# abiswas-odu/Disco

Hardware: AMD Instinct MI355X
Metric: overlaps/sec (BuildGraph stage), 150 bp reads (higher is better)
Workload: dtype u64; 1 GPU; 50000000 x 150 bp synthetic reads, 30x of 50 x 5000000 bp uniform-random contigs, both strands, error-free, min-overlap 40 (k=39), transitive reduction on, seed 42; reads=50000000, read_len=150, min_overlap=40, parallelism=1 GPU, e_pre=903537181, e_out=45314794, n_contained=4685156, cap_bind_sites=0, asymmetric_pairs=0, probes=5550000000, kmer_hits=2220071992

## Files before the change

disco_amd/csrc/disco_hip.hip:

```cpp
#include <hip/hip_runtime.h>
#include <rocprofiler-sdk-roctx/roctx.h>

#include <algorithm>
#include <atomic>
#include <chrono>
#include <cstdarg>
#include <cstdio>
#include <cstdlib>
#include <cstring>
#include <fcntl.h>
#include <sys/mman.h>
#include <sys/stat.h>
#include <unistd.h>
#include <string>
#include <memory>
#include <thread>
#include <map>
#include <mutex>
#include <vector>

#include "../../include/disco_hip.h"
#include "../../include/disco_hip_test.h"
#include "../../include/disco_hip_inspect.h"
#include "disco_kernels.h"
// ... 844 lines not shown
    c->runs_by_pos = false;
    const int nf = v.k - v.m + 1;
    const int lpr = c->S == VERIFY_SW ? runs_lpr_for(c, nf, c->max_len, nloc) : 0;
    if (lpr && nloc) {
        CHK(ensure(c, c->d_runs, nloc * (u64)lpr));
        c->runs_lpr = lpr;
        c->runs_lo = lo;
        c->runs_n = nloc;
        c->runs_by_pos = list != nullptr;
        pl->lpr = lpr;
        pl->nf = nf;
    }
    return DISCO_OK;
}

typedef void (*IndexRunsFn)(DiscoView, u32 *, ulonglong2 *, u32 *, u64, u64, u32 *, u32 *, u32 *, u64 *, u32, u32, const u64 *);
typedef void (*IndexCountFn)(DiscoView, u32 *, ulonglong2 *, u32 *, u64, u64, u32 *, u32 *, u64 *, u32, u32, const u64 *);
struct IndexCountKernel {
    IndexRunsFn runs = nullptr;
    IndexCountFn plain = nullptr;
};
template <bool COUNT, int NF, int NFMAX, bool LONGK>
static IndexCountKernel index_runs_pick(int lpr)
{
    IndexCountKernel k;
    k.runs = lpr == 16 ? index_runs_kernel<COUNT, NF, 1, NFMAX, LONGK> : index_runs_kernel<COUNT, NF, 2, NFMAX, LONGK>;
    return k;
}
template <bool COUNT>
static IndexCountKernel index_count_pick(int nf, int m, int lpr, bool longk, bool long_class)
{
    if (long_class || !lpr) {
        IndexCountKernel k;
        if (long_class) k.plain = longk ? index_count_kernel<COUNT, true, true> : index_count_kernel<COUNT, false, true>;
        else k.plain = longk ? index_count_kernel<COUNT, true> : index_count_kernel<COUNT>;
        return k;
    }
    if (runs_nf_built(nf, m)) switch (nf) {
        case 7: return index_runs_pick<COUNT, 7, 7, false>(lpr);
        case 12: return index_runs_pick<COUNT, 12, 12, false>(lpr);
        case 17: return index_runs_pick<COUNT, 17, 17, false>(lpr);
        case 22: return index_runs_pick<COUNT, 22, 22, false>(lpr);
        default: return index_runs_pick<COUNT, 27, 27, false>(lpr);
        }
    if (longk) return nf <= 48 ? index_runs_pick<COUNT, 0, 48, true>(lpr) : index_runs_pick<COUNT, 0, 64, true>(lpr);
    if (nf <= 8) return index_runs_pick<COUNT, 0, 8, false>(lpr);
    if (nf <= 12) return index_runs_pick<COUNT, 0, 12, false>(lpr);
    if (nf <= 16) return index_runs_pick<COUNT, 0, 16, false>(lpr);
    if (nf <= 24) return index_runs_pick<COUNT, 0, 24, false>(lpr);
    if (nf <= 32) return index_runs_pick<COUNT, 0, 32, false>(lpr);
    if (nf <= 48) return index_runs_pick<COUNT, 0, 48, false>(lpr);
    return index_runs_pick<COUNT, 0, 64, false>(lpr);
}
static IndexCountKernel index_count_pick(bool count, int nf, int m, int lpr, bool longk, bool long_class)
{
    return count ? index_count_pick<true>(nf, m, lpr, longk, long_class) : index_count_pick<false>(nf, m, lpr, longk, long_class);
}

static int index_count_chunk(disco_ctx *c, const DiscoView &v, const IndexCountPlan &pl, bool count, ulonglong2 *rec_base, u64 a, u64 b)
{
    if (b <= a) return DISCO_OK;
    const dim3 grid((unsigned)((b - a + 255) / 256));
    ulonglong2 *rec = rec_base + 2 * (a - pl.lo);
    u32 *oslot = pl.oslot ? pl.oslot + (a - pl.lo) : nullptr;
    u64 *oitem = pl.oitem ? pl.oitem + (a - pl.lo) : nullptr;
    u32 *okey = pl.list ? nullptr : c->d_okey.p;
    const IndexCountKernel k = index_count_pick(count, pl.nf, v.m, pl.lpr, c->k > 64, false);
    if (k.runs) hipLaunchKernelGGL(k.runs, grid, dim3(256), 0, c->stream, v, c->d_bkt, rec, okey, a, b, c->d_runs + (a - pl.lo) * (u64)pl.lpr, pl.ocnt, oslot, oitem, pl.oidbits, pl.oshift, pl.list);
    else hipLaunchKernelGGL(k.plain, grid, dim3(256), 0, c->stream, v, c->d_bkt, rec, okey, a, b, pl.ocnt, oslot, oitem, pl.oidbits, pl.oshift, pl.list);
    HIPCHK(c, hipGetLastError());
    return DISCO_OK;
}

static int index_count_long(disco_ctx *c, const DiscoView &v, const IndexCountPlan &pl, bool count, ulonglong2 *rec, u32 *oslot, u64 x_lo, u64 x_hi)
{
    const dim3 g((unsigned)((x_hi - x_lo + 255) / 256));
    hipLaunchKernelGGL(index_count_pick(count, 0, v.m, 0, c->k > 64, true).plain, g, dim3(256), 0, c->stream, v, c->d_bkt, rec, c->d_okey, x_lo, x_hi, pl.ocnt, oslot, (u64 *)nullptr, 0u, pl.oshift,
                       (const u64 *)nullptr);
    HIPCHK(c, hipGetLastError());
    return DISCO_OK;
}

static bool binned_index_wanted(disco_ctx *c, int logT)
{
    if (getenv("DISCO_NO_BINNED_INDEX") || 2 * c->n >= 0xFFFF0000ull) return false;
    if (logT > BINX_SPAN_BITS && ensure(c, c->d_rec2, 2 * c->n) != DISCO_OK) {
        (void)hipGetLastError();
        c->err.clear();
        return false;
    }
    return true;
}

static int size_bucket_table(disco_ctx *c)
{
    u64 T = 1024;
    int logT = 10;
    double tscale = 2.0;
    if (const char *e = getenv("DISCO_BUCKET_SCALE")) tscale = atof(e);
    while ((double)T < tscale * (double)c->n && logT < 32) {
        T <<= 1;
        logT++;
    }
    c->T = T;
    c->bshift = 64 - logT;
    return logT;
}

static int index_begin(disco_ctx *c)
{
    const int logT = size_bucket_table(c);
    const u64 T = c->T;
    CHK(ensure(c, c->d_bkt, T + 1));
    CHK(ensure(c, c->d_ent, 2 * c->n));
    CHK(ensure(c, c->d_rec, 2 * c->n));
    CHK(ensure(c, c->d_okey, c->n));
    c->adj_imported = false;
    c->binned_index = binned_index_wanted(c, logT);
    if (!c->binned_index) HIPCHK(c, hipMemsetAsync(c->d_bkt, 0, (T + 1) * sizeof(u32), c->stream));
    return DISCO_OK;
}

struct BinxPlan {
    int span = 0, levels = 0, bits[3] = {0, 0, 0};
};
static BinxPlan binx_plan(int logT)
{
    BinxPlan b;
    b.span = std::min(logT, BINX_SPAN_BITS);
    const int prefix = logT - b.span;
    b.levels = (prefix + BINX_MAX_BITS - 1) / BINX_MAX_BITS;
    for (int l = 0; l < b.levels; l++) b.bits[l] = prefix / b.levels + (l < prefix % b.levels ? 1 : 0);
    return b;
}

template <typename R>
static int binx_partition(disco_ctx *c, const char *what, int bits, u32 kshift, u32 total, R *src, R *dst, const R **out, const u32 **part)
{
    const BinxPlan bp = binx_plan(bits);
    const u32 n_part = 1u << (bits - bp.span);
    const u32 tiles = (total + BINX_TILE - 1u) / BINX_TILE;
    u64 hist_len = 1;
    for (int l = 0, done = 0; l < bp.levels; done += bp.bits[l], l++) hist_len = std::max<u64>(hist_len, ((u64)tiles + (1ull << done)) * (1ull << bp.bits[l]) + 1);
    const u64 tab = ((u64)n_part + 1 + 63) & ~63ull;
    CHK(ensure(c, c->d_binx, 4 * tab + hist_len));
    u32 *seg[2] = {c->d_binx.p, c->d_binx.p + tab}, *tb[2] = {c->d_binx.p + 2 * tab, c->d_binx.p + 3 * tab}, *hist = c->d_binx.p + 4 * tab;
    if (getenv("DISCO_VERBOSE"))
        fprintf(stderr, "[disco] binned %s: 2^%d buckets, %u partitions of 2^%d, %d level(s) of %d / %d / %d bits\n", what, bits, n_part, bp.span, bp.levels, bp.bits[0], bp.bits[1], bp.bits[2]);
    u32 pseg = 1, pnb = 1;
    int cur = 0, done = 0;
    for (int l = 0; l < bp.levels; l++) {
        const u32 nseg = 1u << done, nb = 1u << bp.bits[l], shift = kshift + (u32)(bits - done - bp.bits[l]);
        const u32 grid = tiles + nseg;
        const u64 hlen = (u64)grid * nb + 1;
        hipLaunchKernelGGL(binx_segs_kernel, dim3(1), dim3(1024), 0, c->stream, l ? (const u32 *)hist : (const u32 *)nullptr, (const u32 *)tb[cur ^ 1], pseg, pnb, total, seg[cur], tb[cur]);
        HIPCHK(c, hipMemsetAsync(hist, 0, hlen * sizeof(u32), c->stream));
        hipLaunchKernelGGL(binx_hist_kernel<R>, dim3(grid), dim3(BINX_BLOCK), 0, c->stream, (const R *)src, (const u32 *)seg[cur], (const u32 *)tb[cur], nseg, shift, nb, hist);
        CHK((scan_exclusive<u32, u32>(c, hist, hlen, hist, false, nullptr)));
        hipLaunchKernelGGL(binx_scatter_kernel<R>, dim3(grid), dim3(BINX_BLOCK), 0, c->stream, (const R *)src, dst, (const u32 *)seg[cur], (const u32 *)tb[cur], nseg, shift, nb, (const u32 *)hist);
        HIPCHK(c, hipGetLastError());
        std::swap(src, dst);
        pseg = nseg;
        pnb = nb;
        done += bp.bits[l];
        cur ^= 1;
    }
    hipLaunchKernelGGL(binx_segs_kernel, dim3(1), dim3(1024), 0, c->stream, bp.levels ? (const u32 *)hist : (const u32 *)nullptr, (const u32 *)tb[cur ^ 1], pseg, pnb, total, seg[cur],
                       (u32 *)nullptr);
    HIPCHK(c, hipGetLastError());
    *out = src;
    *part = seg[cur];
    return DISCO_OK;
}

static int binned_build_index(disco_ctx *c)
{
    const int logT = 64 - c->bshift;
    const u32 total = (u32)(2 * c->n);
    const ulonglong2 *rec;
    const u32 *part;
    CHK(binx_partition(c, "index build", logT, 32u, total, c->d_rec.p, c->d_rec2.p, &rec, &part));
    const int span = std::min(logT, BINX_SPAN_BITS);
    hipLaunchKernelGGL(binx_build_kernel<ulonglong2>, dim3(1u << (logT - span)), dim3(BINX_BUILD_BLOCK), 0, c->stream, rec, part, (u32)span, 32u, 0u, total, c->T, c->d_bkt.p, c->d_ent.p);
    HIPCHK(c, hipGetLastError());
    return DISCO_OK;
}

static int binned_build_order(disco_ctx *c)
{
    const int bits = c->order_counted_bits;
    const u32 total = (u32)c->n, kshift = 64u - (u32)bits;
    u64 *items = (u64 *)c->d_rec2.p;
    const u64 *rec;
    const u32 *part;
    CHK(binx_partition(c, "grouping", bits, kshift, total, items, items + c->n, &rec, &part));
    const int span = std::min(bits, BINX_SPAN_BITS);
    hipLaunchKernelGGL(binx_build_kernel<u64>, dim3(1u << (bits - span)), dim3(BINX_BUILD_BLOCK), 0, c->stream, rec, part, (u32)span, kshift, (u32)c->order_id_bits, total, (u64)0,
                       (u32 *)nullptr, c->d_order_own.p);
    HIPCHK(c, hipGetLastError());
    return DISCO_OK;
}

static int start_contained_rows(disco_ctx *c, bool grouped)
{
    const u64 nc = c->n_contained;
    if (c->crows_pending && c->crows_n == nc && (!grouped || c->cgrp_pending)) return DISCO_OK;
    const bool have_rows = c->crows_pending && c->crows_n == nc;
    if (!have_rows) c->crows_pending = c->cgrp_pending = false;
    const u64 max_rows = getenv("DISCO_EAGER_ROWS_MAX") ? (u64)atoll(getenv("DISCO_EAGER_ROWS_MAX")) : (16ull << 20);
    if (c->comm || nc == 0 || nc > max_rows || c->n >= (1ull << 31)) return DISCO_OK;
    if (!c->aux_stream) {
        HIPCHK(c, hipStreamCreateWithFlags(&c->aux_stream, hipStreamNonBlocking));
// ... 614 lines not shown
                if (k >= 3) HIPCHK(c, hipStreamWaitEvent(c->copy_stream, c->ev_unpacked[b], 0));
                HIPCHK(c, hipMemcpyAsync(ring, packed + w0, (w1 - w0) * 8, hipMemcpyHostToDevice, c->copy_stream));
                HIPCHK(c, hipEventRecord(c->ev_copied[b], c->copy_stream));
                HIPCHK(c, hipStreamWaitEvent(c->stream, c->ev_copied[b], 0));
                hipLaunchKernelGGL(unpack_reads_kernel, dim3(flat_grid(c, (hi - lo) * (u64)c->S)), dim3(256), 0, c->stream, (const u64 *)ring, ragged ? 0 : (int)stride_words, (const u64 *)woff, w0,
                                   (const u16 *)c->d_len, lo, hi, c->S, classes ? (u32)DISCO_SHORT_MAX : 0xFFFFu, c->d_reads);
                if (classes)
                    hipLaunchKernelGGL(unpack_long_reads_kernel, dim3(flat_grid(c, shape.n_long * ((u64)dstride + 8))), dim3(256), 0, c->stream, (const u64 *)ring, ragged ? 0 : (int)stride_words,
                                       (const u64 *)woff, w0, (const u16 *)c->d_len, lo, hi, (const u32 *)c->d_long_ids, shape.n_long, n, (int)dstride, c->tailb, c->d_full, c->d_reads);
                HIPCHK(c, hipEventRecord(c->ev_unpacked[b], c->stream));
            } else {
                HIPCHK(c, hipMemcpyAsync(c->d_reads + lo * dstride, packed + lo * dstride, (hi - lo) * (u64)dstride * 8, hipMemcpyHostToDevice, c->copy_stream));
                HIPCHK(c, hipEventRecord(c->ev_copied[b], c->copy_stream));
                HIPCHK(c, hipStreamWaitEvent(c->stream, c->ev_copied[b], 0));
            }
            if (eager) CHK(index_count_chunk(c, v, pl, !c->binned_index, c->d_rec, lo, hi));
        }
        HIPCHK(c, hipGetLastError());
        t_issued = lapms();
        if (c->h_len.size() != n) c->h_len.resize(n);
        uint16_t *hl = c->h_len.data();
        parallel_for(n, [&, hl](u64 b0, u64 e0) { memcpy(hl + b0, len + b0, (e0 - b0) * 2); });
        c->h_len_ok = true;
        t_mirror = lapms();
        HIPCHK(c, hipStreamSynchronize(c->copy_stream));
        if (getenv("DISCO_VERBOSE"))
            fprintf(stderr, "[disco] %s: lengths checked %.1f ms, buffers %.1f, chunks issued %.1f, lengths mirrored %.1f, copies done %.1f (%s%s)\n", who, t_scan, t_alloc, t_issued,
                    t_mirror, lapms(), classes ? "two classes of rows" : "one stride", eager ? ", index counted behind the copies" : "");
        if (woff) {
            HIPCHK(c, hipStreamSynchronize(c->stream));
            release(c, woff);
// ... 909 lines not shown
int disco_build_index(disco_ctx *c)
{
    DISCO_TRACE("disco_build_index");
    if (!c) return DISCO_E_ARG;
    if (c->phase < 1) return fail(c, DISCO_E_STATE, "disco_build_index: no reads");
    HIPCHK(c, hipSetDevice(c->device));
    ph_begin(c, DISCO_PH_INDEX);
    if (c->index_counted) {
        c->index_counted = false;
    } else {
        CHK(two_class_convert(c));
        CHK(index_begin(c));
        const DiscoView v = view(c);
        IndexCountPlan pl;
        CHK(index_count_plan(c, v, 0, c->n, &pl));
        CHK(index_count_chunk(c, v, pl, !c->binned_index, c->d_rec, 0, c->n));
        if (c->two_class) CHK(index_count_long(c, v, pl, !c->binned_index, c->d_rec, pl.oslot, 0, c->n_long));
    }
    const bool binned = c->binned_index;
    if (!binned) CHK((scan_exclusive<u32, u32>(c, c->d_bkt, c->T + 1, c->d_bkt, false, nullptr)));
    c->order_ready = false;
    if (c->order_counted && c->order_counted_lo == 0 && c->order_counted_hi == c->n && !c->two_class && !getenv("DISCO_NO_ORDERED_FILL")) {
        const u64 order_buckets = 1ull << c->order_counted_bits;
        CHK(ensure(c, c->d_order_own, c->n));
        ph_end(c, DISCO_PH_INDEX);
        ph_begin(c, DISCO_PH_ORDER);
        if (c->order_items) CHK(binned_build_order(c));
        else {
            CHK((scan_exclusive<u32, u32>(c, c->d_ocnt, order_buckets + 1, c->d_ocnt, false, nullptr)));
            hipLaunchKernelGGL(order_scatter_kernel, dim3(flat_grid(c, c->n)), dim3(256), 0, c->stream, c->d_okey, c->d_oslot, c->d_ocnt, 32u - (u32)c->order_counted_bits, (u64)0, c->n, c->d_len, c->d_order_own);
        }
        ph_end(c, DISCO_PH_ORDER);
// ... 1904 lines not shown
    auto blo_of = [&](u64 g) { return (g * T + G - 1) / G; };
    const u64 blo = blo_of(r), bhi = blo_of(r + 1);
    const bool part = c->part_index;
    if (!part) {
        CHK(ensure(c, c->d_bkt, T + 1));
        CHK(ensure(c, c->d_ent, 2 * c->n));
    }
    CHK(ensure(c, c->d_okey, c->loci ? c->n_alloc : c->n));
    CHK(ensure(c, c->d_rec, std::max<u64>(2 * nloc, 1)));
    c->adj_imported = false;
    ph_begin(c, DISCO_PH_INDEX);
    DiscoView v = view(c);
    IndexCountPlan pl;
    if (c->loci) {
        CHK(index_count_plan(c, v, 0, c->n_own, &pl, c->d_order_own));
        CHK(index_count_chunk(c, v, pl, false, c->d_rec, 0, c->n_own));
    } else {
        CHK(index_count_plan(c, v, c->q_lo, c->q_hi, &pl));
        CHK(index_count_chunk(c, v, pl, false, c->d_rec, c->q_lo, c->q_hi));
        if (c->two_class && nloc) {
            u32 xb[2] = {0, (u32)c->n_long};
            HIPCHK(c, hipMemcpyAsync(&xb[0], c->d_ovf + c->q_lo, sizeof(u32), hipMemcpyDeviceToHost, c->stream));
            if (c->q_hi < c->n) HIPCHK(c, hipMemcpyAsync(&xb[1], c->d_ovf + c->q_hi, sizeof(u32), hipMemcpyDeviceToHost, c->stream));
            HIPCHK(c, hipStreamSynchronize(c->stream));
            if (xb[1] > xb[0]) {
                ulonglong2 *rec_by_id = c->d_rec - 2 * (ptrdiff_t)c->q_lo;
                u32 *oslot_by_id = pl.oslot ? pl.oslot - (ptrdiff_t)c->q_lo : nullptr;
                CHK(index_count_long(c, v, pl, false, rec_by_id, oslot_by_id, xb[0], xb[1]));
            }
        }
    }
    CHK(ensure(c, c->d_x16a, std::max<u64>(2 * nloc, 1)));
    std::vector<u64> scnt, rcnt, matrix;
    RouteByBucket f{logT, G};
    CHK(route_items(c, c->d_rec.p, 2 * nloc, f, c->d_x16a.p, scnt));
    CHK(exchange_counts(c, scnt, rcnt, &matrix));
    const u64 nrec = vsum(rcnt);
    CHK(ensure(c, c->d_x16b, std::max<u64>(nrec, 1)));
    CHK(a2a_items(c, DISCO_X_INDEX_RECORDS, c->d_x16a, scnt, c->d_x16b, rcnt, sizeof(ulonglong2)));
    std::vector<u64> shard((size_t)G, 0);
    for (u32 p = 0; p < G; p++)
        for (u32 q = 0; q < G; q++) shard[q] += matrix[(size_t)p * G + q];
    u64 base = 0;
// ... 1353 lines not shown
```

disco_amd/csrc/disco_kernels.h:

```cpp
#ifndef DISCO_KERNELS_H_
#define DISCO_KERNELS_H_

#include "disco_device.h"
#include "readgen.h"

#define PROBE_ROWCAP 512
#define PROBE_SEGW 128
#define PROBE_SEGP (PROBE_SEGW + 64)
#define PROBE_ACAP 32
#define PROBE_CHUNK 4096
#define ES_MID 1024
#define ES_DUPBITS 11
#define ES_DUPTAB (1 << ES_DUPBITS)
#ifndef ES_CAP
#define ES_CAP 256
#endif
#ifndef TR_CAP
#define TR_CAP 256
#endif
#define TR_CAP_SMALL 128
#define VERIFY_SW 8
#define ORDER_BUCKET(key, shift) (((key) * 0x9E3779B1u) >> (shift))
#define SCAN_ITEMS 16
#define SCAN_BLOCK 256
// ... 187 lines not shown
        if (L <= (u32)min_overlap || L > 32767u || L > (u32)S * 32u) bad++;
        mx = L > mx ? L : mx;
        mn = L < mn ? L : mn;
    }
    if (bad) atomicAdd(&ctr[CTR_BAD_LEN], (u64)bad);
    for (int o = 32; o > 0; o >>= 1) {
        mx = max(mx, (u32)__shfl_down(mx, o));
        mn = min(mn, (u32)__shfl_down(mn, o));
    }
    if ((threadIdx.x & 63) == 0) {
        atomicMax(&ctr[CTR_MAX_LEN], (u64)mx);
        atomicMax(&ctr[CTR_MIN_LEN], (u64)(0xFFFFu - mn));
    }
}

template <bool COUNT, bool LONGK = false, bool LONGCLASS = false>
__global__ void __launch_bounds__(256) index_count_kernel(DiscoView v, u32 *__restrict__ bkt, ulonglong2 *__restrict__ rec, u32 *__restrict__ okey, u64 lo, u64 hi,
                                                          u32 *__restrict__ ocnt, u32 *__restrict__ oslot, u64 *__restrict__ oitem, u32 oidbits, u32 oshift,
                                                          const u64 *__restrict__ list = nullptr)
{
    const u64 x = lo + (u64)blockIdx.x * 256u + threadIdx.x;
    if (x >= hi) return;
    const u64 i = LONGCLASS ? (u64)v.long_ids[x] : x;
    const u64 lw = (!LONGCLASS && list) ? list[x] : 0ull;
    const u64 rid = (!LONGCLASS && list) ? ORDER_ID(lw) : i;
    if (LONGCLASS) lo = 0;
    const int S = LONGCLASS ? v.SL : v.S;
    const u64 *__restrict__ p = LONGCLASS ? v.full + x * (u64)S : v.reads + rid * (u64)S;
    if (!LONGCLASS && v.full && v.len[rid] > DISCO_SHORT_MAX) return;
    const int L = (!LONGCLASS && list) ? ORDER_LEN(lw) : (int)v.len[rid], k = v.k, m = v.m, nf = k - m + 1;
    const int nmm = L - m + 1;
    const int sfx0 = nmm - nf;
    const u64 mask = (1ull << (2 * m)) - 1ull;
// ... 41 lines not shown
        const int ffirst = (int)((k1 >> 1) & 63u), flast = 63 - (int)((k2 >> 1) & 63u);
        int fsel = ffirst;
        if (ffirst == flast)
            rev = k1 & 1u;
        else {
            rev = kmer_is_rev<false, LONGK>(p, S, j0, k);
            fsel = rev ? flast : ffirst;
        }
        t = rev ? (u32)(nf - 1 - fsel) : (u32)fsel;
        return mmer_key(p, S, j0 + fsel, m);
    };
    u32 tp, rp, ts, rs;
    const u64 kp = resolve(k1p, k2p, 0, tp, rp);
    const u64 ks = resolve(k1s, k2s, sfx0, ts, rs);
    const u64 bp = kp >> v.bshift, bs = ks >> v.bshift;
    const u32 sp = COUNT ? atomicAdd(&bkt[bp], 1u) : 0u;
    const u32 ss = COUNT ? atomicAdd(&bkt[bs], 1u) : 0u;
    rec[2 * (i - lo)] = make_ulonglong2((bp << 32) | sp, PAY_MAKE(kp, rid, tp, rp, 0, L));
    rec[2 * (i - lo) + 1] = make_ulonglong2((bs << 32) | ss, PAY_MAKE(ks, LONGCLASS ? v.n + x : rid, ts, rs, 1, L));
}

#define RUNS_M 23
template <bool B>
struct FlagConst {
    static constexpr bool value = B;
};
template <int M>
struct MmerRoll {
    static_assert(M == 0 || (M > 16 && M <= 24 && (M & 1)), "two dwords, the high one partly used; a 24-bit fold in order_hash32<false>");
    const u64 *__restrict__ p;
    int last_word;
    u32 himask, rsh;
    int pos = 0;
    u64 word = 0;
// ... 19 lines not shown
        chi = st ? rhi : fhi;
    }
    __device__ __forceinline__ u32 hash() const { return order_hash32<M == 0>(((u64)chi << 32) | clo); }
    __device__ __forceinline__ u32 strand() const { return st ? 1u : 0u; }
};
#define RUN_W(e) ((u32)(e) >> 7)
#define RUN_DELTA(e) (((u32)(e) >> 1) & 63u)
#define RUN_STRAND(e) ((u32)(e)&1u)
#define OCC_MAKE(slot, e, wend) (((u32)(slot) << 29) | (RUN_STRAND(e) << 23) | (RUN_DELTA(e) << 17) | ((u32)(wend) << 8) | RUN_W(e))
#define OCC_SLOT(d) ((u32)(d) >> 29)
#define OCC_STRAND(d) (((u32)(d) >> 23) & 1u)
#define OCC_DELTA(d) (((u32)(d) >> 17) & 63u)
#define OCC_END(d) (((u32)(d) >> 8) & 0x1FFu)
#define OCC_FIRST(d) ((u32)(d)&0xFFu)

template <bool COUNT, int NF, int NL, int NFMAX = NF, bool LONGK = false>
__global__ void __launch_bounds__(256) index_runs_kernel(DiscoView v, u32 *__restrict__ bkt, ulonglong2 *__restrict__ rec, u32 *__restrict__ okey, u64 lo, u64 hi,
                                                         u32 *__restrict__ runs, u32 *__restrict__ ocnt, u32 *__restrict__ oslot, u64 *__restrict__ oitem, u32 oidbits,
                                                         u32 oshift,
                                                         const u64 *__restrict__ list = nullptr)
{
    static_assert(NF == 0 || NF == NFMAX, "a specialised instantiation holds exactly its window");
    constexpr int CAP = 32 * NL;
    __shared__ u16 s_runs[256 * CAP];
    __shared__ u32 s_x[3 * 256];
    const u32 tid = threadIdx.x;
    for (u32 x = tid; x < 256u * CAP / 2u; x += 256u) ((u32 *)s_runs)[x] = 0xFFFFFFFFu;
    __syncthreads();
    const u64 i = lo + (u64)blockIdx.x * 256u + tid;
    const u64 lw = (list && i < hi) ? list[i] : 0ull;
    const u64 rid = list ? ORDER_ID(lw) : i;
    const bool other_class = i < hi && v.full && v.len[rid] > DISCO_SHORT_MAX;
    if (other_class) s_runs[tid * CAP] = 0xFFFEu;
// ... 82 lines not shown
            const int ffirst = wbase + (int)((k1 >> 1) & 0x7Fu) - j0, flast = wbase + 127 - (int)((k2 >> 1) & 0x7Fu) - j0;
            int fsel = ffirst;
            if (ffirst == flast)
                rev = k1 & 1u;
            else {
                rev = kmer_is_rev<false, LONGK>(p, v.S, j0, k);
                fsel = rev ? flast : ffirst;
            }
            t = rev ? (u32)(nf - 1 - fsel) : (u32)fsel;
            return mmer_key(p, v.S, j0 + fsel, m);
        };
        u32 tp, rp, ts, rs;
        const u64 kp = resolve(P1, P2, 0, 0, tp, rp);
        const u64 ks = resolve(sx[0], sx[256], (int)sx[512], npos, ts, rs);
        const u64 bp = kp >> v.bshift, bs = ks >> v.bshift;
        const u32 sp = COUNT ? atomicAdd(&bkt[bp], 1u) : 0u;
        const u32 ss = COUNT ? atomicAdd(&bkt[bs], 1u) : 0u;
        rec[2 * (i - lo)] = make_ulonglong2((bp << 32) | sp, PAY_MAKE(kp, rid, tp, rp, 0, L));
        rec[2 * (i - lo) + 1] = make_ulonglong2((bs << 32) | ss, PAY_MAKE(ks, rid, ts, rs, 1, L));
    }
    __syncthreads();
#if defined(INDEX_EXP_NORUNS)
    if (tid != 9999u) return;
#endif
    const u64 r0 = (u64)blockIdx.x * 256u;
    const u64 nr = (hi - lo) - r0 < 256u ? (hi - lo) - r0 : 256u;
    u32 *__restrict__ dst = runs + r0 * (CAP / 2);
    for (u32 x = tid; x < (u32)nr * (CAP / 2); x += 256u) dst[x] = ((const u32 *)s_runs)[x];
}

__global__ void index_fill_kernel(u64 n2, const ulonglong2 *__restrict__ rec, const u32 *__restrict__ bkt, u64 *__restrict__ ent)
{
    u64 i = (u64)blockIdx.x * blockDim.x + threadIdx.x;
    for (; i < n2; i += (u64)gridDim.x * blockDim.x) {
// ... 75 lines not shown
    u32 a = 0, b = nseg;
    while (b - a > 1u) {
        const u32 mid = (a + b) >> 1;
        if (tb[mid] <= t) a = mid;
        else b = mid;
    }
    t0 = tb[a];
    nt = tb[a + 1] - t0;
    ti = t - t0;
    const u32 end = seg[a + 1];
    lo = seg[a] + ti * BINX_TILE;
    hi = end - lo > BINX_TILE ? lo + BINX_TILE : end;
    return true;
}

__device__ __forceinline__ u64 binx_key(const ulonglong2 &r) { return r.x; }
__device__ __forceinline__ u64 binx_key(u64 r) { return r; }
#define BINX_DIGIT(key, shift, nb) ((u32)((key) >> (shift)) & ((nb)-1u))

template <typename R>
__global__ void __launch_bounds__(BINX_BLOCK) binx_hist_kernel(const R *__restrict__ rec, const u32 *__restrict__ seg, const u32 *__restrict__ tb, u32 nseg, u32 shift, u32 nb,
                                                               u32 *__restrict__ hist)
{
    __shared__ u32 s_h[1u << BINX_MAX_BITS];
    u32 t0, nt, ti, lo, hi;
    if (!binx_tile(seg, tb, nseg, t0, nt, ti, lo, hi)) return;
    s_h[threadIdx.x] = 0;
    __syncthreads();
    for (u32 i = lo + threadIdx.x; i < hi; i += BINX_BLOCK) atomicAdd(&s_h[BINX_DIGIT(binx_key(rec[i]), shift, nb)], 1u);
    __syncthreads();
    if (threadIdx.x < nb) hist[(u64)nb * t0 + (u64)threadIdx.x * nt + ti] = s_h[threadIdx.x];
}

template <typename R>
__global__ void __launch_bounds__(BINX_BLOCK) binx_scatter_kernel(const R *__restrict__ src, R *__restrict__ dst, const u32 *__restrict__ seg, const u32 *__restrict__ tb,
                                                                  u32 nseg, u32 shift, u32 nb, const u32 *__restrict__ scan)
{
    static_assert(BINX_BLOCK == (1u << BINX_MAX_BITS) && BINX_TILE % BINX_BLOCK == 0, "a thread per bin; whole rounds per tile");
    constexpr u32 PER = BINX_TILE / BINX_BLOCK;
    __shared__ R s_rec[BINX_TILE];
    __shared__ u32 s_cnt[BINX_BLOCK], s_base[BINX_BLOCK], s_w[BINX_BLOCK / 64u];
    const u32 tid = threadIdx.x;
    u32 t0, nt, ti, lo, hi;
    if (!binx_tile(seg, tb, nseg, t0, nt, ti, lo, hi)) return;
    s_cnt[tid] = 0;
    __syncthreads();
    R r[PER];
    u32 rank[PER];
#pragma unroll
    for (u32 j = 0; j < PER; j++) {
        const u32 i = lo + j * BINX_BLOCK + tid;
        if (i < hi) {
            r[j] = src[i];
            rank[j] = atomicAdd(&s_cnt[BINX_DIGIT(binx_key(r[j]), shift, nb)], 1u);
        }
    }
    __syncthreads();
    const u32 cnt = s_cnt[tid];
    u32 incl = cnt;
    for (int o = 1; o < 64; o <<= 1) {
        const u32 y = __shfl_up(incl, o);
        if ((int)(tid & 63u) >= o) incl += y;
    }
    if ((tid & 63u) == 63u) s_w[tid >> 6] = incl;
    __syncthreads();
    u32 start = incl - cnt;
    for (u32 w = 0; w < (tid >> 6); w++) start += s_w[w];
    __syncthreads();
    s_cnt[tid] = start;
    if (tid < nb) s_base[tid] = scan[(u64)nb * t0 + (u64)tid * nt + ti] - start;
    __syncthreads();
#pragma unroll
    for (u32 j = 0; j < PER; j++) {
        const u32 i = lo + j * BINX_BLOCK + tid;
        if (i < hi) s_rec[s_cnt[BINX_DIGIT(binx_key(r[j]), shift, nb)] + rank[j]] = r[j];
    }
    __syncthreads();
    for (u32 j = tid; j < hi - lo; j += BINX_BLOCK) {
        const R x = s_rec[j];
        dst[s_base[BINX_DIGIT(binx_key(x), shift, nb)] + j] = x;
    }
}

__device__ __forceinline__ u64 binx_payload(const ulonglong2 &r, u32, u32) { return r.y; }
__device__ __forceinline__ u64 binx_payload(u64 r, u32 kshift, u32 idbits) { return ORDER_MAKE(r & ((1ull << idbits) - 1ull), (r << (64u - kshift)) >> (64u - kshift + idbits)); }
template <typename R>
__global__ void __launch_bounds__(BINX_BUILD_BLOCK) binx_build_kernel(const R *__restrict__ rec, const u32 *__restrict__ part, u32 span, u32 kshift, u32 idbits, u32 total, u64 T,
                                                                      u32 *__restrict__ bkt, u64 *__restrict__ ent)
{
    constexpr bool TABLE = sizeof(R) == sizeof(ulonglong2);
    __shared__ u32 s_c[1u << BINX_SPAN_BITS];
    __shared__ u32 s_w[16];
    const u32 tid = threadIdx.x, p = blockIdx.x;
    const u32 nbk = 1u << span, mask = nbk - 1u;
    const u32 beg = part[p], end = part[p + 1];
    for (u32 x = tid; x < nbk; x += BINX_BUILD_BLOCK) s_c[x] = 0;
    __syncthreads();
    for (u32 i = beg + tid; i < end; i += BINX_BUILD_BLOCK) atomicAdd(&s_c[(u32)(binx_key(rec[i]) >> kshift) & mask], 1u);
    __syncthreads();
    u32 carry = beg;
    for (u32 base = 0; base < nbk; base += BINX_BUILD_BLOCK) {
        const u32 x = s_c[base + tid];
        u32 sum;
        const u32 ex = binx_block_scan1024(x, s_w, &sum);
        s_c[base + tid] = carry + ex;
        if (TABLE) bkt[(u64)p * nbk + base + tid] = carry + ex;
        carry += sum;
    }
    if (TABLE && (u64)(p + 1u) * nbk == T && tid == 0) bkt[T] = total;
    __syncthreads();
    for (u32 i = beg + tid; i < end; i += BINX_BUILD_BLOCK) {
        const R x = rec[i];
        ent[atomicAdd(&s_c[(u32)(binx_key(x) >> kshift) & mask], 1u)] = binx_payload(x, kshift, idbits);
    }
}

template <typename InT>
__global__ void __launch_bounds__(SCAN_BLOCK) scan_tile_sums_kernel(const InT *__restrict__ in, u64 n, u64 *__restrict__ tile_sums)
{
    __shared__ u64 s_part[SCAN_BLOCK / DISCO_WAVE];
    u64 base = (u64)blockIdx.x * SCAN_TILE;
    u64 sum = 0;
    for (int i = 0; i < SCAN_ITEMS; i++) {
        u64 idx = base + (u64)i * SCAN_BLOCK + threadIdx.x;
        if (idx < n) sum += (u64)in[idx];
    }
    for (int o = 32; o > 0; o >>= 1) sum += __shfl_down(sum, o);
    if ((threadIdx.x & 63) == 0) s_part[threadIdx.x >> 6] = sum;
// ... 3732 lines not shown
```

Before: 11.03 billion overlaps/s.

## Store binned index records as split key/payload planes instead of 16-byte pairs

When the binned index path is active, the index-count kernels now write a u32 bucket key plane and a u64 payload plane in place of 16-byte {key<<32|slot, payload} records. The partition histogram, scatter and build kernels then read only the 4-byte key plane where they need just the key, which cuts memory traffic for the radix partition passes. The record buffers also shrink from 16 to 12 bytes per entry. The build and histogram loops are additionally unrolled to batch loads ahead of the shared-memory atomics. This adds more template plumbing, and the scatter now issues two separate stores per record.

```diff
diff --git a/disco_amd/csrc/disco_hip.hip b/disco_amd/csrc/disco_hip.hip
--- a/disco_amd/csrc/disco_hip.hip
+++ b/disco_amd/csrc/disco_hip.hip
@@ -882,82 +882,136 @@
     return DISCO_OK;
 }
 
-typedef void (*IndexRunsFn)(DiscoView, u32 *, ulonglong2 *, u32 *, u64, u64, u32 *, u32 *, u32 *, u64 *, u32, u32, const u64 *);
-typedef void (*IndexCountFn)(DiscoView, u32 *, ulonglong2 *, u32 *, u64, u64, u32 *, u32 *, u64 *, u32, u32, const u64 *);
+typedef void (*IndexRunsFn)(DiscoView, u32 *, ulonglong2 *, u32 *, u32 *, u64, u64, u32 *, u32 *, u32 *, u64 *, u32, u32, const u64 *);
+typedef void (*IndexCountFn)(DiscoView, u32 *, ulonglong2 *, u32 *, u32 *, u64, u64, u32 *, u32 *, u64 *, u32, u32, const u64 *);
 struct IndexCountKernel {
     IndexRunsFn runs = nullptr;
     IndexCountFn plain = nullptr;
 };
-template <bool COUNT, int NF, int NFMAX, bool LONGK>
+template <int FORM, int NF, int NFMAX, bool LONGK>
 static IndexCountKernel index_runs_pick(int lpr)
 {
     IndexCountKernel k;
-    k.runs = lpr == 16 ? index_runs_kernel<COUNT, NF, 1, NFMAX, LONGK> : index_runs_kernel<COUNT, NF, 2, NFMAX, LONGK>;
+    k.runs = lpr == 16 ? index_runs_kernel<FORM, NF, 1, NFMAX, LONGK> : index_runs_kernel<FORM, NF, 2, NFMAX, LONGK>;
     return k;
 }
-template <bool COUNT>
+template <int FORM>
 static IndexCountKernel index_count_pick(int nf, int m, int lpr, bool longk, bool long_class)
 {
     if (long_class || !lpr) {
         IndexCountKernel k;
-        if (long_class) k.plain = longk ? index_count_kernel<COUNT, true, true> : index_count_kernel<COUNT, false, true>;
-        else k.plain = longk ? index_count_kernel<COUNT, true> : index_count_kernel<COUNT>;
+        if (long_class) k.plain = longk ? index_count_kernel<FORM, true, true> : index_count_kernel<FORM, false, true>;
+        else k.plain = longk ? index_count_kernel<FORM, true> : index_count_kernel<FORM>;
         return k;
     }
     if (runs_nf_built(nf, m)) switch (nf) {
-        case 7: return index_runs_pick<COUNT, 7, 7, false>(lpr);
-        case 12: return index_runs_pick<COUNT, 12, 12, false>(lpr);
-        case 17: return index_runs_pick<COUNT, 17, 17, false>(lpr);
-        case 22: return index_runs_pick<COUNT, 22, 22, false>(lpr);
-        default: return index_runs_pick<COUNT, 27, 27, false>(lpr);
-        }
-    if (longk) return nf <= 48 ? index_runs_pick<COUNT, 0, 48, true>(lpr) : index_runs_pick<COUNT, 0, 64, true>(lpr);
-    if (nf <= 8) return index_runs_pick<COUNT, 0, 8, false>(lpr);
-    if (nf <= 12) return index_runs_pick<COUNT, 0, 12, false>(lpr);
-    if (nf <= 16) return index_runs_pick<COUNT, 0, 16, false>(lpr);
-    if (nf <= 24) return index_runs_pick<COUNT, 0, 24, false>(lpr);
-    if (nf <= 32) return index_runs_pick<COUNT, 0, 32, false>(lpr);
-    if (nf <= 48) return index_runs_pick<COUNT, 0, 48, false>(lpr);
-    return index_runs_pick<COUNT, 0, 64, false>(lpr);
-}
-static IndexCountKernel index_count_pick(bool count, int nf, int m, int lpr, bool longk, bool long_class)
-{
-    return count ? index_count_pick<true>(nf, m, lpr, longk, long_class) : index_count_pick<false>(nf, m, lpr, longk, long_class);
-}
-
-static int index_count_chunk(disco_ctx *c, const DiscoView &v, const IndexCountPlan &pl, bool count, ulonglong2 *rec_base, u64 a, u64 b)
+        case 7: return index_runs_pick<FORM, 7, 7, false>(lpr);
+        case 12: return index_runs_pick<FORM, 12, 12, false>(lpr);
+        case 17: return index_runs_pick<FORM, 17, 17, false>(lpr);
+        case 22: return index_runs_pick<FORM, 22, 22, false>(lpr);
+        default: return index_runs_pick<FORM, 27, 27, false>(lpr);
+        }
+    if (longk) return nf <= 48 ? index_runs_pick<FORM, 0, 48, true>(lpr) : index_runs_pick<FORM, 0, 64, true>(lpr);
+    if (nf <= 8) return index_runs_pick<FORM, 0, 8, false>(lpr);
+    if (nf <= 12) return index_runs_pick<FORM, 0, 12, false>(lpr);
+    if (nf <= 16) return index_runs_pick<FORM, 0, 16, false>(lpr);
+    if (nf <= 24) return index_runs_pick<FORM, 0, 24, false>(lpr);
+    if (nf <= 32) return index_runs_pick<FORM, 0, 32, false>(lpr);
+    if (nf <= 48) return index_runs_pick<FORM, 0, 48, false>(lpr);
+    return index_runs_pick<FORM, 0, 64, false>(lpr);
+}
+static IndexCountKernel index_count_pick(int form, int nf, int m, int lpr, bool longk, bool long_class)
+{
+    switch (form) {
+    case REC_COUNTED: return index_count_pick<REC_COUNTED>(nf, m, lpr, longk, long_class);
+    case REC_ROUTED: return index_count_pick<REC_ROUTED>(nf, m, lpr, longk, long_class);
+    default: return index_count_pick<REC_PLANES>(nf, m, lpr, longk, long_class);
+    }
+}
+
+struct RecOut {
+    int form = REC_COUNTED;
+    ulonglong2 *rec = nullptr;
+    u32 *key = nullptr;
+    RecOut at(ptrdiff_t j) const
+    {
+        RecOut o = *this;
+        if (form == REC_PLANES) {
+            o.rec = (ulonglong2 *)((u64 *)rec + j);
+            o.key = key + j;
+        } else
+            o.rec = rec + j;
+        return o;
+    }
+};
+static RecOut rec_routed(ulonglong2 *rec)
+{
+    RecOut o;
+    o.form = REC_ROUTED;
+    o.rec = rec;
+    return o;
+}
+
+static int index_count_chunk(disco_ctx *c, const DiscoView &v, const IndexCountPlan &pl, const RecOut &out, u64 a, u64 b)
 {
     if (b <= a) return DISCO_OK;
     const dim3 grid((unsigned)((b - a + 255) / 256));
-    ulonglong2 *rec = rec_base + 2 * (a - pl.lo);
+    const RecOut o = out.at((ptrdiff_t)(2 * (a - pl.lo)));
     u32 *oslot = pl.oslot ? pl.oslot + (a - pl.lo) : nullptr;
     u64 *oitem = pl.oitem ? pl.oitem + (a - pl.lo) : nullptr;
     u32 *okey = pl.list ? nullptr : c->d_okey.p;
-    const IndexCountKernel k = index_count_pick(count, pl.nf, v.m, pl.lpr, c->k > 64, false);
-    if (k.runs) hipLaunchKernelGGL(k.runs, grid, dim3(256), 0, c->stream, v, c->d_bkt, rec, okey, a, b, c->d_runs + (a - pl.lo) * (u64)pl.lpr, pl.ocnt, oslot, oitem, pl.oidbits, pl.oshift, pl.list);
-    else hipLaunchKernelGGL(k.plain, grid, dim3(256), 0, c->stream, v, c->d_bkt, rec, okey, a, b, pl.ocnt, oslot, oitem, pl.oidbits, pl.oshift, pl.list);
+    const IndexCountKernel k = index_count_pick(o.form, pl.nf, v.m, pl.lpr, c->k > 64, false);
+    if (k.runs) hipLaunchKernelGGL(k.runs, grid, dim3(256), 0, c->stream, v, c->d_bkt, o.rec, o.key, okey, a, b, c->d_runs + (a - pl.lo) * (u64)pl.lpr, pl.ocnt, oslot, oitem, pl.oidbits, pl.oshift, pl.list);
+    else hipLaunchKernelGGL(k.plain, grid, dim3(256), 0, c->stream, v, c->d_bkt, o.rec, o.key, okey, a, b, pl.ocnt, oslot, oitem, pl.oidbits, pl.oshift, pl.list);
     HIPCHK(c, hipGetLastError());
     return DISCO_OK;
 }
 
-static int index_count_long(disco_ctx *c, const DiscoView &v, const IndexCountPlan &pl, bool count, ulonglong2 *rec, u32 *oslot, u64 x_lo, u64 x_hi)
+static int index_count_long(disco_ctx *c, const DiscoView &v, const IndexCountPlan &pl, const RecOut &out, u32 *oslot, u64 x_lo, u64 x_hi)
 {
     const dim3 g((unsigned)((x_hi - x_lo + 255) / 256));
-    hipLaunchKernelGGL(index_count_pick(count, 0, v.m, 0, c->k > 64, true).plain, g, dim3(256), 0, c->stream, v, c->d_bkt, rec, c->d_okey, x_lo, x_hi, pl.ocnt, oslot, (u64 *)nullptr, 0u, pl.oshift,
+    hipLaunchKernelGGL(index_count_pick(out.form, 0, v.m, 0, c->k > 64, true).plain, g, dim3(256), 0, c->stream, v, c->d_bkt, out.rec, out.key, c->d_okey, x_lo, x_hi, pl.ocnt, oslot, (u64 *)nullptr, 0u, pl.oshift,
                        (const u64 *)nullptr);
     HIPCHK(c, hipGetLastError());
     return DISCO_OK;
 }
 
+template <typename R>
+struct BinxSide {
+    typename R::Key *key = nullptr;
+    u64 *pay = nullptr;
+};
+static u64 binx_plane_elems(u64 n) { return (3 * n + 1) / 2; }
+static BinxSide<BinxPlanes> binx_side(ulonglong2 *buf, u64 n)
+{
+    BinxSide<BinxPlanes> s;
+    if (!buf) return s;
+    s.pay = (u64 *)buf;
+    s.key = (u32 *)(s.pay + 2 * n);
+    return s;
+}
 static bool binned_index_wanted(disco_ctx *c, int logT)
 {
     if (getenv("DISCO_NO_BINNED_INDEX") || 2 * c->n >= 0xFFFF0000ull) return false;
-    if (logT > BINX_SPAN_BITS && ensure(c, c->d_rec2, 2 * c->n) != DISCO_OK) {
+    if (logT > BINX_SPAN_BITS && ensure(c, c->d_rec2, binx_plane_elems(c->n)) != DISCO_OK) {
         (void)hipGetLastError();
         c->err.clear();
         return false;
     }
     return true;
+}
+
+static RecOut index_records(disco_ctx *c)
+{
+    RecOut o;
+    if (c->binned_index) {
+        const BinxSide<BinxPlanes> s = binx_side(c->d_rec.p, c->n);
+        o.form = REC_PLANES;
+        o.rec = (ulonglong2 *)s.pay;
+        o.key = s.key;
+    } else
+        o.rec = c->d_rec.p;
+    return o;
 }
 
 static int size_bucket_table(disco_ctx *c)
@@ -981,10 +1035,10 @@
     const u64 T = c->T;
     CHK(ensure(c, c->d_bkt, T + 1));
     CHK(ensure(c, c->d_ent, 2 * c->n));
-    CHK(ensure(c, c->d_rec, 2 * c->n));
     CHK(ensure(c, c->d_okey, c->n));
     c->adj_imported = false;
     c->binned_index = binned_index_wanted(c, logT);
+    CHK(ensure(c, c->d_rec, c->binned_index ? binx_plane_elems(c->n) : 2 * c->n));
     if (!c->binned_index) HIPCHK(c, hipMemsetAsync(c->d_bkt, 0, (T + 1) * sizeof(u32), c->stream));
     return DISCO_OK;
 }
@@ -1003,8 +1057,9 @@
 }
 
 template <typename R>
-static int binx_partition(disco_ctx *c, const char *what, int bits, u32 kshift, u32 total, R *src, R *dst, const R **out, const u32 **part)
-{
+static int binx_partition(disco_ctx *c, const char *what, int bits, u32 kshift, u32 total, BinxSide<R> src, BinxSide<R> dst, BinxSide<R> *out, const u32 **part)
+{
+    typedef typename R::Key Key;
     const BinxPlan bp = binx_plan(bits);
     const u32 n_part = 1u << (bits - bp.span);
     const u32 tiles = (total + BINX_TILE - 1u) / BINX_TILE;
@@ -1023,9 +1078,10 @@
         const u64 hlen = (u64)grid * nb + 1;
         hipLaunchKernelGGL(binx_segs_kernel, dim3(1), dim3(1024), 0, c->stream, l ? (const u32 *)hist : (const u32 *)nullptr, (const u32 *)tb[cur ^ 1], pseg, pnb, total, seg[cur], tb[cur]);
         HIPCHK(c, hipMemsetAsync(hist, 0, hlen * sizeof(u32), c->stream));
-        hipLaunchKernelGGL(binx_hist_kernel<R>, dim3(grid), dim3(BINX_BLOCK), 0, c->stream, (const R *)src, (const u32 *)seg[cur], (const u32 *)tb[cur], nseg, shift, nb, hist);
+        hipLaunchKernelGGL(binx_hist_kernel<R>, dim3(grid), dim3(BINX_BLOCK), 0, c->stream, (const Key *)src.key, (const u32 *)seg[cur], (const u32 *)tb[cur], nseg, shift, nb, hist);
         CHK((scan_exclusive<u32, u32>(c, hist, hlen, hist, false, nullptr)));
-        hipLaunchKernelGGL(binx_scatter_kernel<R>, dim3(grid), dim3(BINX_BLOCK), 0, c->stream, (const R *)src, dst, (const u32 *)seg[cur], (const u32 *)tb[cur], nseg, shift, nb, (const u32 *)hist);
+        hipLaunchKernelGGL(binx_scatter_kernel<R>, dim3(grid), dim3(BINX_BLOCK), 0, c->stream, (const Key *)src.key, (const u64 *)src.pay, dst.key, dst.pay, (const u32 *)seg[cur], (const u32 *)tb[cur],
+                           nseg, shift, nb, (const u32 *)hist);
         HIPCHK(c, hipGetLastError());
         std::swap(src, dst);
         pseg = nseg;
@@ -1045,11 +1101,12 @@
 {
     const int logT = 64 - c->bshift;
     const u32 total = (u32)(2 * c->n);
-    const ulonglong2 *rec;
+    BinxSide<BinxPlanes> rec;
     const u32 *part;
-    CHK(binx_partition(c, "index build", logT, 32u, total, c->d_rec.p, c->d_rec2.p, &rec, &part));
+    CHK(binx_partition<BinxPlanes>(c, "index build", logT, 0u, total, binx_side(c->d_rec.p, c->n), binx_side(c->d_rec2.p, c->n), &rec, &part));
     const int span = std::min(logT, BINX_SPAN_BITS);
-    hipLaunchKernelGGL(binx_build_kernel<ulonglong2>, dim3(1u << (logT - span)), dim3(BINX_BUILD_BLOCK), 0, c->stream, rec, part, (u32)span, 32u, 0u, total, c->T, c->d_bkt.p, c->d_ent.p);
+    hipLaunchKernelGGL(binx_build_kernel<BinxPlanes>, dim3(1u << (logT - span)), dim3(BINX_BUILD_BLOCK), 0, c->stream, (const u32 *)rec.key, (const u64 *)rec.pay, part, (u32)span, 0u, 0u, total, c->T,
+                       c->d_bkt.p, c->d_ent.p);
     HIPCHK(c, hipGetLastError());
     return DISCO_OK;
 }
@@ -1058,12 +1115,14 @@
 {
     const int bits = c->order_counted_bits;
     const u32 total = (u32)c->n, kshift = 64u - (u32)bits;
-    u64 *items = (u64 *)c->d_rec2.p;
-    const u64 *rec;
+    BinxSide<BinxItems> items, other, rec;
+    items.key = (u64 *)c->d_rec2.p;
+    other.key = items.key + c->n;
     const u32 *part;
-    CHK(binx_partition(c, "grouping", bits, kshift, total, items, items + c->n, &rec, &part));
+    CHK(binx_partition<BinxItems>(c, "grouping", bits, kshift, total, items, other, &rec, &part));
     const int span = std::min(bits, BINX_SPAN_BITS);
-    hipLaunchKernelGGL(binx_build_kernel<u64>, dim3(1u << (bits - span)), dim3(BINX_BUILD_BLOCK), 0, c->stream, rec, part, (u32)span, kshift, (u32)c->order_id_bits, total, (u64)0,
+    hipLaunchKernelGGL(binx_build_kernel<BinxItems>, dim3(1u << (bits - span)), dim3(BINX_BUILD_BLOCK), 0, c->stream, (const u64 *)rec.key, (const u64 *)nullptr, part, (u32)span, kshift,
+                       (u32)c->order_id_bits, total, (u64)0,
                        (u32 *)nullptr, c->d_order_own.p);
     HIPCHK(c, hipGetLastError());
     return DISCO_OK;
@@ -1708,7 +1767,7 @@
                 HIPCHK(c, hipEventRecord(c->ev_copied[b], c->copy_stream));
                 HIPCHK(c, hipStreamWaitEvent(c->stream, c->ev_copied[b], 0));
             }
-            if (eager) CHK(index_count_chunk(c, v, pl, !c->binned_index, c->d_rec, lo, hi));
+            if (eager) CHK(index_count_chunk(c, v, pl, index_records(c), lo, hi));
         }
         HIPCHK(c, hipGetLastError());
         t_issued = lapms();
@@ -2648,8 +2707,8 @@
         const DiscoView v = view(c);
         IndexCountPlan pl;
         CHK(index_count_plan(c, v, 0, c->n, &pl));
-        CHK(index_count_chunk(c, v, pl, !c->binned_index, c->d_rec, 0, c->n));
-        if (c->two_class) CHK(index_count_long(c, v, pl, !c->binned_index, c->d_rec, pl.oslot, 0, c->n_long));
+        CHK(index_count_chunk(c, v, pl, index_records(c), 0, c->n));
+        if (c->two_class) CHK(index_count_long(c, v, pl, index_records(c), pl.oslot, 0, c->n_long));
     }
     const bool binned = c->binned_index;
     if (!binned) CHK((scan_exclusive<u32, u32>(c, c->d_bkt, c->T + 1, c->d_bkt, false, nullptr)));
@@ -4584,10 +4643,10 @@
     IndexCountPlan pl;
     if (c->loci) {
         CHK(index_count_plan(c, v, 0, c->n_own, &pl, c->d_order_own));
-        CHK(index_count_chunk(c, v, pl, false, c->d_rec, 0, c->n_own));
+        CHK(index_count_chunk(c, v, pl, rec_routed(c->d_rec), 0, c->n_own));
     } else {
         CHK(index_count_plan(c, v, c->q_lo, c->q_hi, &pl));
-        CHK(index_count_chunk(c, v, pl, false, c->d_rec, c->q_lo, c->q_hi));
+        CHK(index_count_chunk(c, v, pl, rec_routed(c->d_rec), c->q_lo, c->q_hi));
         if (c->two_class && nloc) {
             u32 xb[2] = {0, (u32)c->n_long};
             HIPCHK(c, hipMemcpyAsync(&xb[0], c->d_ovf + c->q_lo, sizeof(u32), hipMemcpyDeviceToHost, c->stream));
@@ -4596,7 +4655,7 @@
             if (xb[1] > xb[0]) {
                 ulonglong2 *rec_by_id = c->d_rec - 2 * (ptrdiff_t)c->q_lo;
                 u32 *oslot_by_id = pl.oslot ? pl.oslot - (ptrdiff_t)c->q_lo : nullptr;
-                CHK(index_count_long(c, v, pl, false, rec_by_id, oslot_by_id, xb[0], xb[1]));
+                CHK(index_count_long(c, v, pl, rec_routed(rec_by_id), oslot_by_id, xb[0], xb[1]));
             }
         }
     }
diff --git a/disco_amd/csrc/disco_kernels.h b/disco_amd/csrc/disco_kernels.h
--- a/disco_amd/csrc/disco_kernels.h
+++ b/disco_amd/csrc/disco_kernels.h
@@ -225,9 +225,24 @@
     }
 }
 
-template <bool COUNT, bool LONGK = false, bool LONGCLASS = false>
-__global__ void __launch_bounds__(256) index_count_kernel(DiscoView v, u32 *__restrict__ bkt, ulonglong2 *__restrict__ rec, u32 *__restrict__ okey, u64 lo, u64 hi,
-                                                          u32 *__restrict__ ocnt, u32 *__restrict__ oslot, u64 *__restrict__ oitem, u32 oidbits, u32 oshift,
+enum { REC_COUNTED = 0, REC_ROUTED = 1, REC_PLANES = 2 };
+template <int FORM>
+__device__ __forceinline__ void index_put_records(u32 *__restrict__ bkt, ulonglong2 *__restrict__ rec, u32 *__restrict__ rkey, u64 j, u64 b0, u64 p0, u64 b1, u64 p1)
+{
+    if (FORM == REC_PLANES) {
+        *(uint2 *)(rkey + j) = make_uint2((u32)b0, (u32)b1);
+        *(ulonglong2 *)((u64 *)rec + j) = make_ulonglong2(p0, p1);
+    } else {
+        const u32 s0 = FORM == REC_COUNTED ? atomicAdd(&bkt[b0], 1u) : 0u;
+        const u32 s1 = FORM == REC_COUNTED ? atomicAdd(&bkt[b1], 1u) : 0u;
+        rec[j] = make_ulonglong2((b0 << 32) | s0, p0);
+        rec[j + 1] = make_ulonglong2((b1 << 32) | s1, p1);
+    }
+}
+
+template <int FORM, bool LONGK = false, bool LONGCLASS = false>
+__global__ void __launch_bounds__(256) index_count_kernel(DiscoView v, u32 *__restrict__ bkt, ulonglong2 *__restrict__ rec, u32 *__restrict__ rkey, u32 *__restrict__ okey, u64 lo,
+                                                          u64 hi, u32 *__restrict__ ocnt, u32 *__restrict__ oslot, u64 *__restrict__ oitem, u32 oidbits, u32 oshift,
                                                           const u64 *__restrict__ list = nullptr)
 {
     const u64 x = lo + (u64)blockIdx.x * 256u + threadIdx.x;
@@ -299,10 +314,7 @@
     const u64 kp = resolve(k1p, k2p, 0, tp, rp);
     const u64 ks = resolve(k1s, k2s, sfx0, ts, rs);
     const u64 bp = kp >> v.bshift, bs = ks >> v.bshift;
-    const u32 sp = COUNT ? atomicAdd(&bkt[bp], 1u) : 0u;
-    const u32 ss = COUNT ? atomicAdd(&bkt[bs], 1u) : 0u;
-    rec[2 * (i - lo)] = make_ulonglong2((bp << 32) | sp, PAY_MAKE(kp, rid, tp, rp, 0, L));
-    rec[2 * (i - lo) + 1] = make_ulonglong2((bs << 32) | ss, PAY_MAKE(ks, LONGCLASS ? v.n + x : rid, ts, rs, 1, L));
+    index_put_records<FORM>(bkt, rec, rkey, 2 * (i - lo), bp, PAY_MAKE(kp, rid, tp, rp, 0, L), bs, PAY_MAKE(ks, LONGCLASS ? v.n + x : rid, ts, rs, 1, L));
 }
 
 #define RUNS_M 23
@@ -352,9 +364,9 @@
 #define OCC_END(d) (((u32)(d) >> 8) & 0x1FFu)
 #define OCC_FIRST(d) ((u32)(d)&0xFFu)
 
-template <bool COUNT, int NF, int NL, int NFMAX = NF, bool LONGK = false>
-__global__ void __launch_bounds__(256) index_runs_kernel(DiscoView v, u32 *__restrict__ bkt, ulonglong2 *__restrict__ rec, u32 *__restrict__ okey, u64 lo, u64 hi,
-                                                         u32 *__restrict__ runs, u32 *__restrict__ ocnt, u32 *__restrict__ oslot, u64 *__restrict__ oitem, u32 oidbits,
+template <int FORM, int NF, int NL, int NFMAX = NF, bool LONGK = false>
+__global__ void __launch_bounds__(256) index_runs_kernel(DiscoView v, u32 *__restrict__ bkt, ulonglong2 *__restrict__ rec, u32 *__restrict__ rkey, u32 *__restrict__ okey, u64 lo,
+                                                         u64 hi, u32 *__restrict__ runs, u32 *__restrict__ ocnt, u32 *__restrict__ oslot, u64 *__restrict__ oitem, u32 oidbits,
                                                          u32 oshift,
                                                          const u64 *__restrict__ list = nullptr)
 {
@@ -467,10 +479,7 @@
         const u64 kp = resolve(P1, P2, 0, 0, tp, rp);
         const u64 ks = resolve(sx[0], sx[256], (int)sx[512], npos, ts, rs);
         const u64 bp = kp >> v.bshift, bs = ks >> v.bshift;
-        const u32 sp = COUNT ? atomicAdd(&bkt[bp], 1u) : 0u;
-        const u32 ss = COUNT ? atomicAdd(&bkt[bs], 1u) : 0u;
-        rec[2 * (i - lo)] = make_ulonglong2((bp << 32) | sp, PAY_MAKE(kp, rid, tp, rp, 0, L));
-        rec[2 * (i - lo) + 1] = make_ulonglong2((bs << 32) | ss, PAY_MAKE(ks, rid, ts, rs, 1, L));
+        index_put_records<FORM>(bkt, rec, rkey, 2 * (i - lo), bp, PAY_MAKE(kp, rid, tp, rp, 0, L), bs, PAY_MAKE(ks, rid, ts, rs, 1, L));
     }
     __syncthreads();
 #if defined(INDEX_EXP_NORUNS)
@@ -576,45 +585,95 @@
     return true;
 }
 
-__device__ __forceinline__ u64 binx_key(const ulonglong2 &r) { return r.x; }
-__device__ __forceinline__ u64 binx_key(u64 r) { return r; }
+struct BinxItems {
+    typedef u64 Key;
+    typedef u64 Rec;
+    static constexpr bool TABLE = false;
+    struct Stage {
+        u64 w[BINX_TILE];
+    };
+    static __device__ __forceinline__ Rec load(const Key *__restrict__ key, const u64 *__restrict__, u32 i) { return key[i]; }
+    static __device__ __forceinline__ void store(Key *__restrict__ key, u64 *__restrict__, u32 i, Rec r) { key[i] = r; }
+    static __device__ __forceinline__ Key key_of(Rec r) { return r; }
+    static __device__ __forceinline__ void put(Stage &s, u32 j, Rec r) { s.w[j] = r; }
+    static __device__ __forceinline__ Rec get(const Stage &s, u32 j) { return s.w[j]; }
+    static __device__ __forceinline__ u64 payload(Rec r, u32 kshift, u32 idbits) { return ORDER_MAKE(r & ((1ull << idbits) - 1ull), (r << (64u - kshift)) >> (64u - kshift + idbits)); }
+};
+struct BinxPlanes {
+    typedef u32 Key;
+    struct Rec {
+        u64 pay;
+        u32 key;
+    };
+    static constexpr bool TABLE = true;
+    struct Stage {
+        u64 pay[BINX_TILE];
+        u32 key[BINX_TILE];
+    };
+    static __device__ __forceinline__ Rec load(const Key *__restrict__ key, const u64 *__restrict__ pay, u32 i) { return Rec{pay[i], key[i]}; }
+    static __device__ __forceinline__ void store(Key *__restrict__ key, u64 *__restrict__ pay, u32 i, Rec r)
+    {
+        key[i] = r.key;
+        pay[i] = r.pay;
+    }
+    static __device__ __forceinline__ Key key_of(const Rec &r) { return r.key; }
+    static __device__ __forceinline__ void put(Stage &s, u32 j, const Rec &r)
+    {
+        s.key[j] = r.key;
+        s.pay[j] = r.pay;
+    }
+    static __device__ __forceinline__ Rec get(const Stage &s, u32 j) { return Rec{s.pay[j], s.key[j]}; }
+    static __device__ __forceinline__ u64 payload(const Rec &r, u32, u32) { return r.pay; }
+};
 #define BINX_DIGIT(key, shift, nb) ((u32)((key) >> (shift)) & ((nb)-1u))
 
 template <typename R>
-__global__ void __launch_bounds__(BINX_BLOCK) binx_hist_kernel(const R *__restrict__ rec, const u32 *__restrict__ seg, const u32 *__restrict__ tb, u32 nseg, u32 shift, u32 nb,
-                                                               u32 *__restrict__ hist)
-{
+__global__ void __launch_bounds__(BINX_BLOCK) binx_hist_kernel(const typename R::Key *__restrict__ key, const u32 *__restrict__ seg, const u32 *__restrict__ tb, u32 nseg, u32 shift,
+                                                               u32 nb, u32 *__restrict__ hist)
+{
+    constexpr u32 PER = BINX_TILE / BINX_BLOCK;
     __shared__ u32 s_h[1u << BINX_MAX_BITS];
     u32 t0, nt, ti, lo, hi;
     if (!binx_tile(seg, tb, nseg, t0, nt, ti, lo, hi)) return;
     s_h[threadIdx.x] = 0;
     __syncthreads();
-    for (u32 i = lo + threadIdx.x; i < hi; i += BINX_BLOCK) atomicAdd(&s_h[BINX_DIGIT(binx_key(rec[i]), shift, nb)], 1u);
+    typename R::Key k[PER];
+#pragma unroll
+    for (u32 j = 0; j < PER; j++) {
+        const u32 i = lo + j * BINX_BLOCK + threadIdx.x;
+        if (i < hi) k[j] = key[i];
+    }
+#pragma unroll
+    for (u32 j = 0; j < PER; j++) {
+        const u32 i = lo + j * BINX_BLOCK + threadIdx.x;
+        if (i < hi) atomicAdd(&s_h[BINX_DIGIT(k[j], shift, nb)], 1u);
+    }
     __syncthreads();
     if (threadIdx.x < nb) hist[(u64)nb * t0 + (u64)threadIdx.x * nt + ti] = s_h[threadIdx.x];
 }
 
 template <typename R>
-__global__ void __launch_bounds__(BINX_BLOCK) binx_scatter_kernel(const R *__restrict__ src, R *__restrict__ dst, const u32 *__restrict__ seg, const u32 *__restrict__ tb,
-                                                                  u32 nseg, u32 shift, u32 nb, const u32 *__restrict__ scan)
+__global__ void __launch_bounds__(BINX_BLOCK) binx_scatter_kernel(const typename R::Key *__restrict__ skey, const u64 *__restrict__ spay, typename R::Key *__restrict__ dkey,
+                                                                  u64 *__restrict__ dpay, const u32 *__restrict__ seg, const u32 *__restrict__ tb, u32 nseg, u32 shift, u32 nb,
+                                                                  const u32 *__restrict__ scan)
 {
     static_assert(BINX_BLOCK == (1u << BINX_MAX_BITS) && BINX_TILE % BINX_BLOCK == 0, "a thread per bin; whole rounds per tile");
     constexpr u32 PER = BINX_TILE / BINX_BLOCK;
-    __shared__ R s_rec[BINX_TILE];
+    __shared__ typename R::Stage s_rec;
     __shared__ u32 s_cnt[BINX_BLOCK], s_base[BINX_BLOCK], s_w[BINX_BLOCK / 64u];
     const u32 tid = threadIdx.x;
     u32 t0, nt, ti, lo, hi;
     if (!binx_tile(seg, tb, nseg, t0, nt, ti, lo, hi)) return;
     s_cnt[tid] = 0;
     __syncthreads();
-    R r[PER];
+    typename R::Rec r[PER];
     u32 rank[PER];
 #pragma unroll
     for (u32 j = 0; j < PER; j++) {
         const u32 i = lo + j * BINX_BLOCK + tid;
         if (i < hi) {
-            r[j] = src[i];
-            rank[j] = atomicAdd(&s_cnt[BINX_DIGIT(binx_key(r[j]), shift, nb)], 1u);
+            r[j] = R::load(skey, spay, i);
+            rank[j] = atomicAdd(&s_cnt[BINX_DIGIT(R::key_of(r[j]), shift, nb)], 1u);
         }
     }
     __syncthreads();
@@ -635,22 +694,21 @@
 #pragma unroll
     for (u32 j = 0; j < PER; j++) {
         const u32 i = lo + j * BINX_BLOCK + tid;
-        if (i < hi) s_rec[s_cnt[BINX_DIGIT(binx_key(r[j]), shift, nb)] + rank[j]] = r[j];
+        if (i < hi) R::put(s_rec, s_cnt[BINX_DIGIT(R::key_of(r[j]), shift, nb)] + rank[j], r[j]);
     }
     __syncthreads();
     for (u32 j = tid; j < hi - lo; j += BINX_BLOCK) {
-        const R x = s_rec[j];
-        dst[s_base[BINX_DIGIT(binx_key(x), shift, nb)] + j] = x;
-    }
-}
-
-__device__ __forceinline__ u64 binx_payload(const ulonglong2 &r, u32, u32) { return r.y; }
-__device__ __forceinline__ u64 binx_payload(u64 r, u32 kshift, u32 idbits) { return ORDER_MAKE(r & ((1ull << idbits) - 1ull), (r << (64u - kshift)) >> (64u - kshift + idbits)); }
+        const typename R::Rec x = R::get(s_rec, j);
+        R::store(dkey, dpay, s_base[BINX_DIGIT(R::key_of(x), shift, nb)] + j, x);
+    }
+}
+
 template <typename R>
-__global__ void __launch_bounds__(BINX_BUILD_BLOCK) binx_build_kernel(const R *__restrict__ rec, const u32 *__restrict__ part, u32 span, u32 kshift, u32 idbits, u32 total, u64 T,
-                                                                      u32 *__restrict__ bkt, u64 *__restrict__ ent)
-{
-    constexpr bool TABLE = sizeof(R) == sizeof(ulonglong2);
+__global__ void __launch_bounds__(BINX_BUILD_BLOCK) binx_build_kernel(const typename R::Key *__restrict__ key, const u64 *__restrict__ pay, const u32 *__restrict__ part, u32 span,
+                                                                      u32 kshift, u32 idbits, u32 total, u64 T, u32 *__restrict__ bkt, u64 *__restrict__ ent)
+{
+    constexpr bool TABLE = R::TABLE;
+    constexpr u32 U = 4;
     __shared__ u32 s_c[1u << BINX_SPAN_BITS];
     __shared__ u32 s_w[16];
     const u32 tid = threadIdx.x, p = blockIdx.x;
@@ -658,7 +716,15 @@
     const u32 beg = part[p], end = part[p + 1];
     for (u32 x = tid; x < nbk; x += BINX_BUILD_BLOCK) s_c[x] = 0;
     __syncthreads();
-    for (u32 i = beg + tid; i < end; i += BINX_BUILD_BLOCK) atomicAdd(&s_c[(u32)(binx_key(rec[i]) >> kshift) & mask], 1u);
+    for (u32 b = beg + tid; b < end; b += U * BINX_BUILD_BLOCK) {
+        typename R::Key k[U];
+#pragma unroll
+        for (u32 u = 0; u < U; u++)
+            if (b + u * BINX_BUILD_BLOCK < end) k[u] = key[b + u * BINX_BUILD_BLOCK];
+#pragma unroll
+        for (u32 u = 0; u < U; u++)
+            if (b + u * BINX_BUILD_BLOCK < end) atomicAdd(&s_c[(u32)(k[u] >> kshift) & mask], 1u);
+    }
     __syncthreads();
     u32 carry = beg;
     for (u32 base = 0; base < nbk; base += BINX_BUILD_BLOCK) {
@@ -671,9 +737,14 @@
     }
     if (TABLE && (u64)(p + 1u) * nbk == T && tid == 0) bkt[T] = total;
     __syncthreads();
-    for (u32 i = beg + tid; i < end; i += BINX_BUILD_BLOCK) {
-        const R x = rec[i];
-        ent[atomicAdd(&s_c[(u32)(binx_key(x) >> kshift) & mask], 1u)] = binx_payload(x, kshift, idbits);
+    for (u32 b = beg + tid; b < end; b += U * BINX_BUILD_BLOCK) {
+        typename R::Rec x[U];
+#pragma unroll
+        for (u32 u = 0; u < U; u++)
+            if (b + u * BINX_BUILD_BLOCK < end) x[u] = R::load(key, pay, b + u * BINX_BUILD_BLOCK);
+#pragma unroll
+        for (u32 u = 0; u < U; u++)
+            if (b + u * BINX_BUILD_BLOCK < end) ent[atomicAdd(&s_c[(u32)(R::key_of(x[u]) >> kshift) & mask], 1u)] = R::payload(x[u], kshift, idbits);
     }
 }
 
```

Measured after the change: 11.14 billion overlaps/s (median of 6 runs). No clear change (+0.9%).
